# pairlab/leibnizgym

Measured on AMD Instinct MI355X. Metric: env-steps/sec (whole node), trifinger_difficulty_4 @65536 envs, 1/2/4/8 GPUs, higher is better.
Workload: dtype f32

## Files before the change

### leibnizgym_amd/csrc/tf_roles.h

```cpp
#pragma once
#include <type_traits>

#include "tf_contact.h"

#define NT 256

enum { M_ACT_IN = 1, M_RESETS = 2, M_TORQUE = 4, M_SIM = 8, M_POST = 16, M_FINISH = 32, M_ACT_RAND = 64  };
#define M_FUSED_STEP (M_ACT_IN | M_RESETS | M_TORQUE | M_SIM | M_POST | M_FINISH)
#define M_FUSED_STEP_RAND (M_FUSED_STEP | M_ACT_RAND)
#define M_FUSED_RESET (M_RESETS | M_TORQUE | M_SIM | M_POST)

#define L_REC(f) (30 * (f))
#define R_A 0
#define R_DIR 6
#define R_RXD 15
#define R_U 24
#define R_DL 27
#define P_AW 0
#define P_BW 3
#define P_MINV 6
#define P_S1 12
#define P_C1 13
#define P_P2 14
#define P_P3 17
#define P_VQ 20
#define L_POSE_A 23
#define L_POSE_B 53
#define L_WALL 90
#define L_PARK(f) L_REC(f)
#define PK_FC 0
#define PK_LINK 4
#define PK_TF 5
#define PK_TW 8
#define PK_TAU 11
#define PK_FT 14
#define L_VQFF 138
#define L_INIT 147
#define L_DR0 32
#define LDS_SLOTS 159
DEV constexpr int ffm_mbox(int fd, int k, bool boxw = false) {
    return boxw ? 180 + 6 * fd + k
         : fd == 0 ? (k == 0 ? 147 : 149 + k)
         : fd == 1 ? (k == 0 ? 148 : (k == 1 ? 59 : 153 + k))
                   : 83 + k;
}
#define NT_HELP 512
#define L_HELP_OWN 159
#define L_HELP_DR 177
#define LDS_SLOTS_HELP 180
DEV constexpr int ffm_own_mbox(int fm, int k) { return L_HELP_OWN + 6 * fm + k; }
#define L_POSE_S 150
#define LDS_SLOTS_BOX 159
#define LDS_SLOTS_BOX_WIDE 198
#define L_CONE 180
#define LDS_SLOTS_SURF 268
#define L_XCH (MAX_STATES)
#define L_NAN (MAX_STATES + 18)
#define L_VSQ (MAX_STATES + 22)
#define L_OTERM (MAX_STATES + 31)
static_assert(MAX_STATES + 37 <= LDS_SLOTS, "post-phase LDS map");
#define LD(slot) lds[(slot) * WAVE + lane]

struct Ctx {
    int tid, lane, role;
    int wave_first, i, n_valid;
    bool valid;
};

#define ST_RSRC() __builtin_amdgcn_make_buffer_rsrc((void*)P.state, 0, TF_STATE_ROWS * P.N * 4, 0x00020000)
#define LDST(row) __builtin_bit_cast(float, __builtin_amdgcn_raw_buffer_load_b32(ST_RSRC(), (unsigned)cx.i * 4u, (row) * P.N * 4, 0))
#define STST(row, val) do { if (cx.valid) __builtin_amdgcn_raw_buffer_store_b32(__builtin_bit_cast(unsigned, (float)(val)), ST_RSRC(), (unsigned)cx.i * 4u, (row) * P.N * 4, 0); } while (0)
#define BAR() __syncthreads()
#define IN_FLIGHT3(a, b, c) asm volatile("" : "+v"(a), "+v"(b), "+v"(c))
#define IN_FLIGHT4(a, b, c, d) asm volatile("" : "+v"(a), "+v"(b), "+v"(c), "+v"(d))

#ifdef TF_PHASE_TIMING
#define TF_SCR_STRIDE 256
#define NOW() ((uint32_t)__builtin_readcyclecounter())
#define STAMP(id) do { if (cx.lane == 0) ((gu32*)P.scratch)[((size_t)blockIdx.x * 4 + cx.role) * 64 + (id)] = NOW(); } while (0)
#define STAMPV(id, val) do { if (cx.lane == 0) ((gu32*)P.scratch)[((size_t)blockIdx.x * 4 + cx.role) * 64 + (id)] = (uint32_t)(val); } while (0)
#else
#define TF_SCR_STRIDE 16
#define NOW() 0u
#define STAMP(id) do { } while (0)
#define STAMPV(id, val) do { } while (0)
#endif

#define NT_F 192
template <int W, int NTH = NT>
DEV void coop_store_tile(gfloat* __restrict__ dst, const float* lds, const Ctx& cx) {
    const unsigned total = (unsigned)(cx.n_valid * W);
    gfloat* base = dst + (size_t)cx.wave_first * (size_t)W;
    const unsigned total4 = total >> 2;
    const __amdgpu_buffer_rsrc_t tile = __builtin_amdgcn_make_buffer_rsrc((void*)base, 0, (int)(total4 * 16u), 0x00020000);
    constexpr int ITER = (16 * W + NTH - 1) / NTH;
    const unsigned last4 = total4 - 1u;
#pragma unroll
    for (int k = 0; k < ITER; ++k) {
        const unsigned idx = (unsigned)cx.tid + (unsigned)(NTH * k);
        const unsigned src = (idx < last4) ? idx : last4;
        u32x4 vv = *reinterpret_cast<const u32x4*>(&lds[src * 4u]);
        __builtin_amdgcn_raw_buffer_store_b128(vv, tile, idx * 16u, 0, 0);
    }
    const unsigned tail = (total4 << 2) + (unsigned)cx.tid;
    if (tail < total) base[tail] = lds[tail];
}
template <int W, int LS, int NTH = NT>
DEV void coop_store_tile_strided(gfloat* __restrict__ dst, const float* lds, const Ctx& cx) {
    const unsigned total = (unsigned)(cx.n_valid * W);
    gfloat* base = dst + (size_t)cx.wave_first * (size_t)W;
    const unsigned total4 = total >> 2;
    const __amdgpu_buffer_rsrc_t tile = __builtin_amdgcn_make_buffer_rsrc((void*)base, 0, (int)(total4 * 16u), 0x00020000);
    constexpr int ITER = (16 * W + NTH - 1) / NTH;
    const unsigned lastf = total - 1u;
#pragma unroll
    for (int k = 0; k < ITER; ++k) {
        const unsigned idx = (unsigned)cx.tid + (unsigned)(NTH * k);
        u32x4 vv;
#pragma unroll
        for (int e = 0; e < 4; ++e) {
            unsigned g = idx * 4u + (unsigned)e;
            g = (g < lastf) ? g : lastf;
            const unsigned row = g / (unsigned)W, col = g - row * (unsigned)W;
            vv[e] = __builtin_bit_cast(unsigned, lds[row * (unsigned)LS + col]);
        }
        __builtin_amdgcn_raw_buffer_store_b128(vv, tile, idx * 16u, 0, 0);
    }
    const unsigned tail = (total4 << 2) + (unsigned)cx.tid;
    if (tail < total) { const unsigned row = tail / (unsigned)W, col = tail - row * (unsigned)W; base[tail] = lds[row * (unsigned)LS + col]; }
}
template <int A>
DEV void coop_load_tile(const float* __restrict__ src, float* lds, const Ctx& cx) {
    const float* base = src + (size_t)cx.wave_first * (size_t)A;
    const unsigned last = (unsigned)(cx.n_valid * A) - 1u;
    constexpr int ITER = (WAVE * A + NT - 1) / NT;
    float t[ITER];
#pragma unroll
    for (int k = 0; k < ITER; ++k) {
        const unsigned idx = (unsigned)cx.tid + (unsigned)(NT * k);
        t[k] = base[idx < last ? idx : last];
    }
#pragma unroll
    for (int k = 0; k < ITER; ++k) {
        const unsigned idx = (unsigned)cx.tid + (unsigned)(NT * k);
        if (idx < (unsigned)(WAVE * A)) lds[idx] = t[k];
    }
}

template <int A>
DEV void draw_action_tile(const DevParams& P, const StepArgs& sa, float* lds, const Ctx& cx) {
    constexpr int NB = (A + 3) / 4;
    for (int t = cx.tid; t < WAVE * NB; t += NT) {
        const int e = t / NB, b = t - e * NB;
        const int ge = cx.wave_first + ((e < cx.n_valid) ? e : (cx.n_valid - 1));
        float u[4];
        rng4(P, (uint32_t)(P.env_id_offset + ge), sa.frame0, RNG_ACTION + (uint32_t)b, u);
#pragma unroll
        for (int k = 0; k < 4; ++k) {
            const int c = 4 * b + k;
            if (c < A) lds[e * A + c] = 2.0f * u[k] - 1.0f;
        }
    }
}

DEV void sample_xy(float u_r, float u_t, float r_max, float& x, float& y) {
    float radius = f_sqrt(u_r) * r_max;
    float s, c;
    tf_sincos(6.2831855f * u_t, s, c);
    x = radius * c;
    y = radius * s;
}
DEV void sample_yaw_quat(float u, float q[4]) {
    float s, c;
    tf_sincos((6.2831855f * u) * 0.5f, s, c);
    q[0] = 0.0f; q[1] = 0.0f; q[2] = s; q[3] = c;
}
DEV void normalize_quat(const float n[4], float q[4]) {
    float nrm = f_sqrt(n[0] * n[0] + n[1] * n[1] + n[2] * n[2] + n[3] * n[3]);
    float inv = 1.0f / f_max(nrm, 1e-12f);
#pragma unroll
    for (int i = 0; i < 4; ++i) q[i] = n[i] * inv;
}

DEV void sample_goal_pos(const DevParams& P, uint32_t gid, uint32_t count, float xyz[3], float quat[4]) {
    const int d = P.task_difficulty;
    float u[4];
    rng4(P, gid, count, RNG_GOAL_POS, u);
    float x = 0.0f, y = 0.0f, z;
    quat[0] = 0.0f; quat[1] = 0.0f; quat[2] = 0.0f; quat[3] = 1.0f;
    if (d == -1 || d == 1 || d == 3 || d == 4 || d == 5) sample_xy(u[0], u[1], P.m.obj_max_com_dist, x, y);
    if (d == -1 || d == 1) z = P.m.obj_min_height;
    else if (d == 2 || d == 6) z = P.m.obj_min_height + 0.05f;
    else if (d == 3) z = P.m.obj_span_min_height * u[2] + P.m.obj_min_height;
    else z = P.m.obj_span_radius * u[2] + P.m.obj_radius_3d;
    if (d == -1) sample_yaw_quat(u[3], quat);
    xyz[0] = x; xyz[1] = y; xyz[2] = z;
}
DEV bool goal_has_random_quat(const DevParams& P) { const int d = P.task_difficulty; return d == 4 || d == 5 || d == 6; }
DEV void sample_goal_rot(const DevParams& P, uint32_t gid, uint32_t count, float quat[4], float gw[3]) {
    if (goal_has_random_quat(P)) {
        float v[4], n[4];
        rng4(P, gid, count, RNG_GOAL_QUAT, v);
        box_muller(v[0], v[1], n[0], n[1]);
        box_muller(v[2], v[3], n[2], n[3]);
        normalize_quat(n, quat);
    }
    if (P.goal_rotation_activate) {
        float v[4], n[4];
        rng4(P, gid, count, RNG_GOAL_ANGVEL, v);
        box_muller(v[0], v[1], n[0], n[1]);
        box_muller(v[2], v[3], n[2], n[3]);
        float nrm = f_sqrt(n[0] * n[0] + n[1] * n[1] + n[2] * n[2]);
        float mag = n[3] * P.goal_rate;
#pragma unroll
        for (int i = 0; i < 3; ++i) gw[i] = mag * (n[i] / nrm);
    } else {
        gw[0] = 0.0f; gw[1] = 0.0f; gw[2] = 0.0f;
    }
}
template <bool EXT>
DEV void goal_from_raw(const float raw[10], const float dr[TF_NUM_DR], float gp[3], float gq[4], float gw[3]) {
    gp[0] = EXT ? raw[0] + dr[TF_DR_STAGE_POS] : raw[0]; gp[1] = EXT ? raw[1] + dr[TF_DR_STAGE_POS + 1] : raw[1]; gp[2] = raw[2];
#pragma unroll
    for (int i = 0; i < 4; ++i) gq[i] = raw[3 + i];
#pragma unroll
    for (int i = 0; i < 3; ++i) gw[i] = raw[7 + i];
}
template <bool EXT>
DEV void sample_goal(const DevParams& P, uint32_t gid, uint32_t count, const float dr[TF_NUM_DR], float gp[3], float gq[4], float gw[3]) {
    float raw[10];
    sample_goal_pos(P, gid, count, &raw[0], &raw[3]);
    sample_goal_rot(P, gid, count, &raw[3], &raw[7]);
    goal_from_raw<EXT>(raw, dr, gp, gq, gw);
}

template <bool EXT>
DEV void draw_dr(const DevParams& P, uint32_t gid, uint32_t count, float dr[TF_NUM_DR]) {
    float u[4];
    rng4(P, gid, count, RNG_DR, u);
    dr[0] = FMA(P.dr_cube_mass[1] - P.dr_cube_mass[0], u[0], P.dr_cube_mass[0]);
    dr[1] = FMA(P.dr_cube_size[1] - P.dr_cube_size[0], u[1], P.dr_cube_size[0]);
    dr[2] = FMA(P.dr_friction[1] - P.dr_friction[0], u[2], P.dr_friction[0]);
    dr[3] = FMA(P.dr_motor[1] - P.dr_motor[0], u[3], P.dr_motor[0]);
    rng4(P, gid, count, RNG_DR + 1u, u);
    dr[4] = FMA(P.dr_link_mass[1] - P.dr_link_mass[0], u[0], P.dr_link_mass[0]);
    dr[5] = FMA(P.dr_restitution[1] - P.dr_restitution[0], u[1], P.dr_restitution[0]);
    if (!EXT) return;
    rng4(P, gid, count, RNG_DR + 2u, u);
#pragma unroll
    for (int k = 0; k < 3; ++k) dr[TF_DR_BASE_POS + k] = P.dr_base_pos[k] * (2.0f * u[k] - 1.0f);
    dr[TF_DR_STAGE_POS] = P.dr_stage_pos[0] * (2.0f * u[3] - 1.0f);
    rng4(P, gid, count, RNG_DR + 3u, u);
    dr[TF_DR_STAGE_POS + 1] = P.dr_stage_pos[1] * (2.0f * u[0] - 1.0f);
    dr[TF_DR_FRICTION_ROBOT] = FMA(P.dr_friction_robot[1] - P.dr_friction_robot[0], u[1], P.dr_friction_robot[0]);
    dr[TF_DR_FRICTION_OBJECT] = FMA(P.dr_friction_object[1] - P.dr_friction_object[0], u[2], P.dr_friction_object[0]);
    dr[TF_DR_FRICTION_STAGE] = FMA(P.dr_friction_stage[1] - P.dr_friction_stage[0], u[3], P.dr_friction_stage[0]);
}
DEV float pair_factor(float mu_a, float fa1, float mu_b, float fb1) {
    const float inv = 1.0f / (mu_a + mu_b);
    return FMA(mu_b * inv, fb1, FMA(mu_a * inv, fa1, 1.0f));
}

DEV float emit_scaled(float x, float lo, float hi, bool nrm, float co) {
    const float o_ = (lo + hi) * 0.5f, i_ = 1.0f / (hi - lo);
    return f_clamp(nrm ? FMA(x, 2.0f * i_, -(2.0f * o_) * i_) : x, -co, co);
}
DEV float emit_table(const DevParams& P, int col, float x, bool nrm, float co) {
    const float off = P.tables[TAB_OFF + col], inv = P.tables[TAB_INV + col];
    return f_clamp(nrm ? FMA(x, 2.0f * inv, -(2.0f * off) * inv) : x, -co, co);
}
#define QLO(j) (((j) % 3 == 0) ? -0.33f : (((j) % 3 == 1) ? 0.0f : -2.7f))
#define QHI(j) (((j) % 3 == 0) ? 1.0f : (((j) % 3 == 1) ? 1.57f : 0.0f))
#define PLO(j) (((j) == 2) ? 0.0f : -0.3f)
#define TLO(j) (((j) < 2) ? -0.4f : (((j) == 2) ? 0.0f : (((j) < 7) ? -1.0f : -0.2f)))
#define THI(j) (((j) < 2) ? 0.4f : (((j) == 2) ? 0.5f : (((j) < 7) ? 1.0f : 0.2f)))

DEV float norm3d(const float a[3], const float b[3]) {
    float dx = a[0] - b[0], dy = a[1] - b[1], dz = a[2] - b[2];
    return f_sqrt(dx * dx + dy * dy + dz * dz);
}
DEV float ipow(float x, int n) {
    float t = x;
    for (int k = 1; k < n; ++k) t = t * x;
    return t;
}
DEV float norm_p3(const float a[3], const float b[3], int p) {
    if (__builtin_expect(p == 2, 1)) return norm3d(a, b);
    const float ax = f_abs(a[0] - b[0]), ay = f_abs(a[1] - b[1]), az = f_abs(a[2] - b[2]);
    if (p == 1) return (ax + ay) + az;
    if (p == TF_NORM_INF) return f_max(f_max(ax, ay), az);
    const float mx = f_max(f_max(ax, ay), az);
    if (!(mx > 0.0f)) return 0.0f;
    const float s = (ipow(ax / mx, p) + ipow(ay / mx, p)) + ipow(az / mx, p);
    float y = tf_exp(tf_log(s) / (float)p);
    const float yp1 = ipow(y, p - 1);
    y = y - (yp1 * y - s) / ((float)p * yp1);
    return mx * y;
}

DEV void tip_state(const DevModel& m, const Yaw& y, const FK& k, const float q[3], const float qd[3], float out[13]) {
    float To[3];
    link_point<3>(k, m.tip_origin, To);
    base_to_world(y, To, &out[0]);
    float sy, cy, sx, cxx;
    tf_sincos(0.5f * q[0], sy, cy);
    tf_sincos(0.5f * (q[1] + q[2]), sx, cxx);
    float qyx[4] = {cy * sx, sy * cxx, -(sy * sx), cy * cxx};
    float qz[4] = {0.0f, 0.0f, y.hs, y.hc};
    quat_mul(qz, qyx, &out[3]);
    float L1[3], L2[3], L3[3], vb[3], wb[3];
    levers(k, To, L1, L2, L3);
#pragma unroll
    for (int i = 0; i < 3; ++i) vb[i] = L1[i] * qd[0] + L2[i] * qd[1] + L3[i] * qd[2];
    wb[0] = k.ax[0] * qd[1] + k.ax[0] * qd[2];
    wb[1] = qd[0];
    wb[2] = k.ax[2] * qd[1] + k.ax[2] * qd[2];
    dir_base_to_world(y, vb, &out[7]);
    dir_base_to_world(y, wb, &out[10]);
}

struct FingerPubRegs { FK k; };
DEV void read_pub(const float* lds, int lane, int f, FingerPubRegs& p) {
    const int pb = L_REC(f);
#pragma unroll
    for (int j = 0; j < 3; ++j) { p.k.p2[j] = LD(pb + P_P2 + j); p.k.p3[j] = LD(pb + P_P3 + j); }
#pragma unroll
    for (int j = 0; j < 6; ++j) p.k.Minv[j] = LD(pb + P_MINV + j);
    p.k.s1 = LD(pb + P_S1); p.k.c1 = LD(pb + P_C1);
    p.k.ax[0] = p.k.c1; p.k.ax[1] = 0.0f; p.k.ax[2] = -p.k.s1;
}

struct TipContact {
    bool active;
    float J[9], Dinv[3], bias, lam[3], mu;
    float arm[3];
};

template <int A, bool IS_RESET, bool ASYM, int MODE, int X, bool WIDE, bool HELP = false, bool DR = true>
DEV void finger_role(const DevParams& P, const StepArgs& sa, const float* __restrict__ action, float* lds, const Ctx& cx) {
    static_assert(!HELP || WIDE, "helper wavefronts: 256-register kernels only");
    constexpr bool EXT = X != 0;
    constexpr bool BOXK = X == 2;
    const DevModel& m = P.m;
    const int f = cx.role, lane = cx.lane;
    constexpr int OD = TF_OBS_DIM_BASE + A, SD = OD + TF_STATES_EXTRA;
    constexpr int TW = ASYM ? SD : OD;
    constexpr int NDR = EXT ? TF_NUM_DR : TF_DR_BASE_POS;
    constexpr int AJ = A / 3;
    const Yaw yw = {m.base_yaw_cos[f], m.base_yaw_sin[f], m.base_half_yaw_cos[f], m.base_half_yaw_sin[f], m.base_height};
    const uint32_t gid = (uint32_t)(P.env_id_offset + cx.i);
    float q[3], qd[3], tau[3], dr[TF_NUM_DR];
    uint8_t fl_reset = 0;
    uint32_t fl_count = 0;
// ... 1109 lines not shown
struct StatsTicket { unsigned long long mine, old; };
DEV void stats_begin(const DevParams& P, const LaneStats& st, int lane, StatsTicket& tk) {
    float vals[11];
#pragma unroll
    for (int t = 0; t < 6; ++t) vals[t] = st.rew[t];
    vals[6] = st.pos_cnt; vals[7] = st.ori_cnt; vals[8] = st.succ; vals[9] = st.resets; vals[10] = st.nonfinite;
    float sum = 0.0f;
#pragma unroll
    for (int k = 0; k < 11; ++k) {
        const float s = wave_sum_lane63(vals[k]);
        const float b = __builtin_bit_cast(float, __builtin_amdgcn_readlane(__builtin_bit_cast(int, s), WAVE - 1));
        sum = (lane == k) ? b : sum;
    }
    const long long fx = (long long)((double)sum * STAT_FIX);
    tk.mine = ((unsigned long long)fx << STAT_COUNT_BITS) + 1ull;
    tk.old = 0ull;
    const int shard = (int)blockIdx.x & (STAT_SHARDS - 1);
    gu64* acc = (gu64*)P.tickets;
    if (lane < 11)
        tk.old = __hip_atomic_fetch_add(&acc[(shard * 11 + lane) * STAT_STRIDE], tk.mine, __ATOMIC_RELAXED, __HIP_MEMORY_SCOPE_AGENT);
}
DEV void stats_end(const DevParams& P, int lane, const StatsTicket& tk) {
    const unsigned long long cmask = (1ull << STAT_COUNT_BITS) - 1ull;
    const int nw = (int)gridDim.x;
    const int shard = (int)blockIdx.x & (STAT_SHARDS - 1);
    const unsigned long long members = (unsigned long long)((nw - shard + STAT_SHARDS - 1) / STAT_SHARDS);
    const unsigned long long nshards = (unsigned long long)(nw < STAT_SHARDS ? nw : STAT_SHARDS);
    gu64* acc = (gu64*)P.tickets;
    if (lane < 11 && (tk.old & cmask) == members - 1ull) {
        const unsigned long long total1 = tk.old + tk.mine;
        __hip_atomic_store(&acc[(shard * 11 + lane) * STAT_STRIDE], 0ull, __ATOMIC_RELAXED, __HIP_MEMORY_SCOPE_AGENT);
        const unsigned long long v2 = (total1 & ~cmask) + 1ull;
        gu64* top = &acc[(STAT_SHARDS * 11 + lane) * STAT_STRIDE];
        const unsigned long long old2 = __hip_atomic_fetch_add(top, v2, __ATOMIC_RELAXED, __HIP_MEMORY_SCOPE_AGENT);
        if ((old2 & cmask) == nshards - 1ull) {
            __hip_atomic_store(top, 0ull, __ATOMIC_RELAXED, __HIP_MEMORY_SCOPE_AGENT);
            const long long fxs = (long long)(old2 + v2) >> STAT_COUNT_BITS;
            const float total = (float)((double)fxs / STAT_FIX);
            const int k = lane;
            const float o = (k < 6 || k == 8) ? total / (float)P.N : total;
            const int slot = (k < 6) ? k : ((k == 6) ? TF_INFO_POS_COUNT : ((k == 7) ? TF_INFO_ORI_COUNT :
                             ((k == 8) ? TF_INFO_SUCCESS_MEAN : ((k == 9) ? TF_INFO_NUM_RESETS : TF_INFO_NUM_NONFINITE))));
            P.info[slot] = o;
        }
    }
}

DEV void stats_zero(LaneStats& st) {
#pragma unroll
    for (int t = 0; t < 6; ++t) st.rew[t] = 0.0f;
    st.pos_cnt = 0.0f; st.ori_cnt = 0.0f; st.succ = 0.0f; st.resets = 0.0f; st.nonfinite = 0.0f;
}


DEV void ld_row(const float* lds, int lane, int rb, float2v rec[3]) {
#pragma unroll
    for (int j = 0; j < 3; ++j) { rec[j].x = LD(rb + j); rec[j].y = LD(rb + 3 + j); }
}
DEV float pk_row_vel_lds(const float* lds, int lane, int rb, const Twist& t) { float2v rec[3]; ld_row(lds, lane, rb, rec); return pk_row_vel(rec, t); }
DEV void pk_row_apply_lds(const float* lds, int lane, int rb, float dl, float2v mI, Twist& t) { float2v rec[3]; ld_row(lds, lane, rb, rec); pk_row_apply(rec, dl, mI, t); }

DEV void wall_arms(bool box, const float* lds, int lane, const float r[3], const float n[2], float a[3], float b[3], float c3[3]) {
    wall_arm_n(r, n, a);
    wall_arm_t(r, n, b);
    c3[0] = 0.0f; c3[1] = 0.0f; c3[2] = 0.0f;
    if (__builtin_expect(box, 0)) {
        float S[6], t[3], ez[3];
#pragma unroll
        for (int e = 0; e < 6; ++e) S[e] = LD(L_POSE_S + e);
        sym3_mul(S, a, t); a[0] = t[0]; a[1] = t[1]; a[2] = t[2];
        sym3_mul(S, b, t); b[0] = t[0]; b[1] = t[1]; b[2] = t[2];
        box_axis(0, ez);
        box_arm(S, r, ez, c3);
    }
}

template <int A, bool IS_RESET, bool ASYM, int MODE, int X, bool WIDE, bool HELP = false, bool SURF = false, bool DR = true>
DEV void cube_role(const DevParams& P, const StepArgs& sa, const float* __restrict__ action, float* lds, const Ctx& cx) {
    constexpr bool EXT = X != 0;
    constexpr bool BOXK = X == 2;
    static_assert(!SURF || (WIDE && !BOXK), "the surface normal of the cube corners is built into the 256-register cube kernels only");
    const DevModel& m = P.m;
    const int lane = cx.lane;
    constexpr int OD = TF_OBS_DIM_BASE + A, SD = OD + TF_STATES_EXTRA;
    constexpr int TW = ASYM ? SD : OD;
    constexpr int NDR = EXT ? TF_NUM_DR : TF_DR_BASE_POS;
    const uint32_t gid = (uint32_t)(P.env_id_offset + cx.i);
    float cp[3], cq[4], cv[3], cw[3], dr[TF_NUM_DR];
    float lam_cf[12], lam_cw[12], cf_face = 0.0f, cw_face = 0.0f;
    uint8_t fl_reset = 0, fl_goal_reset = 0, fl_successes = 0;
    int fl_steps = 0;
    uint32_t fl_count = 0;
    STAMP(0);
#pragma unroll
    for (int j = 0; j < 3; ++j) { cp[j] = LDST(TF_S_CUBE_P + j); cv[j] = LDST(TF_S_CUBE_V + j); cw[j] = LDST(TF_S_CUBE_W + j); }
#pragma unroll
    for (int j = 0; j < 4; ++j) cq[j] = LDST(TF_S_CUBE_Q + j);
#pragma unroll
    for (int j = 0; j < TF_NUM_DR; ++j) dr[j] = (DR && j < NDR && P.dr_enable) ? LDST(TF_S_DR + j) : TF_DR_NEUTRAL(j);
    if (MODE & (M_RESETS | M_POST | M_FINISH)) {
        fl_reset = P.reset_buf[(unsigned)cx.i];
        fl_goal_reset = P.goal_reset_buf[(unsigned)cx.i];
        fl_successes = P.successes[(unsigned)cx.i];
        fl_steps = (int)P.steps[(unsigned)cx.i];
        fl_count = P.reset_count[(unsigned)cx.i];
    }
    if (MODE & M_ACT_RAND) draw_action_tile<A>(P, sa, lds, cx);
    else if (MODE & M_ACT_IN) coop_load_tile<A>(action, lds, cx);
    else if (MODE & (M_RESETS | M_TORQUE | M_POST)) coop_load_tile<A>((const float*)P.action_buf, lds, cx);
    if (DR && P.dr_enable) {
#pragma unroll
        for (int j = 0; j < NDR; ++j) LD(L_DR0 + j) = dr[j];
    }
    BAR();
    if (!(MODE & (M_ACT_IN | M_RESETS))) BAR();
    STAMP(1);
    if (MODE & (M_SIM | M_RESETS)) {
        cf_face = LDST(TF_S_CF_FACE); cw_face = LDST(TF_S_CW_FACE);
#pragma unroll
        for (int j = 0; j < 12; ++j) { lam_cf[j] = LDST(TF_S_LAM_CF + j); lam_cw[j] = 0.0f; }
        const bool cw_was = cw_face != 0.0f;
        if (__builtin_amdgcn_ballot_w64(cw_was) != 0ull) {
#pragma unroll
            for (int j = 0; j < 12; ++j) { const float t = LDST(TF_S_LAM_CW + j); lam_cw[j] = cw_was ? t : 0.0f; }
        }
    }
    bool c_reset = fl_reset != 0, c_goal_reset = fl_goal_reset != 0, c_successes = fl_successes != 0;
    int c_steps = fl_steps;
    float n_resets = 0.0f;
    if (MODE & M_RESETS) {
        const bool rflag = IS_RESET || (fl_reset != 0);
        const bool gflag = !IS_RESET && (fl_goal_reset != 0);
        uint32_t count = fl_count;
        float gp[3] = {0.0f, 0.0f, 0.0f}, gq[4] = {0.0f, 0.0f, 0.0f, 0.0f}, gw[3] = {0.0f, 0.0f, 0.0f};
        float nx_obj[4] = {0.0f, 0.0f, 0.0f, 0.0f}, nx_goal[10] = {0.0f, 0.0f, 0.0f, 0.0f, 0.0f, 0.0f, 0.0f, 0.0f, 0.0f, 0.0f};
        bool have = false;
        if (!IS_RESET && __builtin_amdgcn_ballot_w64(rflag) != 0ull) {
            const uint32_t tag = __builtin_bit_cast(uint32_t, LDST(TF_S_NEXT_TAG));
            have = rflag && (tag == count + 1u);
#pragma unroll
            for (int j = 0; j < 4; ++j) nx_obj[j] = LDST(TF_S_NEXT_OBJ + j);
#pragma unroll
            for (int j = 0; j < 10; ++j) nx_goal[j] = LDST(TF_S_NEXT_GOAL + j);
        }
        const bool draw_now = __builtin_amdgcn_ballot_w64(rflag && !have) != 0ull;
        if (rflag) {
            if (DR && P.dr_enable) draw_dr<EXT>(P, gid, count, dr);
            if (P.object_reset_type == TF_RESET_DEFAULT) {
                cp[0] = EXT ? 0.0f + dr[TF_DR_STAGE_POS] : 0.0f; cp[1] = EXT ? 0.0f + dr[TF_DR_STAGE_POS + 1] : 0.0f; cp[2] = m.obj_min_height * dr[1];
                cq[0] = 0.0f; cq[1] = 0.0f; cq[2] = 0.0f; cq[3] = 1.0f;
#pragma unroll
                for (int k = 0; k < 3; ++k) { cv[k] = 0.0f; cw[k] = 0.0f; }
            } else if (P.object_reset_type == TF_RESET_RANDOM) {
                float ox = nx_obj[0], oy = nx_obj[1], oq[4] = {0.0f, 0.0f, nx_obj[2], nx_obj[3]};
                if (draw_now) {
                    float u[4], tx, ty, tq[4];
                    rng4(P, gid, count, RNG_OBJECT, u);
                    sample_xy(u[0], u[1], m.obj_max_com_dist, tx, ty);
                    sample_yaw_quat(u[2], tq);
                    ox = have ? ox : tx; oy = have ? oy : ty; oq[2] = have ? oq[2] : tq[2]; oq[3] = have ? oq[3] : tq[3];
                }
                cp[0] = EXT ? ox + dr[TF_DR_STAGE_POS] : ox; cp[1] = EXT ? oy + dr[TF_DR_STAGE_POS + 1] : oy;
                cp[2] = m.obj_min_height * dr[1];
#pragma unroll
                for (int k = 0; k < 4; ++k) cq[k] = oq[k];
#pragma unroll
                for (int k = 0; k < 3; ++k) { cv[k] = 0.0f; cw[k] = 0.0f; }
            }
            if (draw_now) {
                float raw[10];
                sample_goal_pos(P, gid, count, &raw[0], &raw[3]);
                sample_goal_rot(P, gid, count, &raw[3], &raw[7]);
#pragma unroll
                for (int j = 0; j < 10; ++j) nx_goal[j] = have ? nx_goal[j] : raw[j];
            }
            goal_from_raw<EXT>(nx_goal, dr, gp, gq, gw);
            count = count + 1u;
#pragma unroll
            for (int j = 0; j < 12; ++j) { lam_cf[j] = 0.0f; lam_cw[j] = 0.0f; }
            cf_face = 0.0f; cw_face = 0.0f;
            n_resets = cx.valid ? 1.0f : 0.0f;
        }
        if (gflag) {
            sample_goal<EXT>(P, gid, count, dr, gp, gq, gw);
            count = count + 1u;
        }
        if (cx.valid) {
            if (rflag) { P.reset_buf[(unsigned)cx.i] = 0; P.steps[(unsigned)cx.i] = 0; P.successes[(unsigned)cx.i] = 0; }
            if (gflag) P.goal_reset_buf[(unsigned)cx.i] = 0;
            if (rflag || gflag) P.reset_count[(unsigned)cx.i] = count;
        }
        if (DR && rflag && P.dr_enable) {
#pragma unroll
            for (int j = 0; j < NDR; ++j) STST(TF_S_DR + j, dr[j]);
        }
        if (rflag || gflag) {
#pragma unroll
            for (int j = 0; j < 3; ++j) { STST(TF_S_GOAL_P + j, gp[j]); STST(TF_S_GOAL_W + j, gw[j]); }
#pragma unroll
            for (int j = 0; j < 4; ++j) STST(TF_S_GOAL_Q + j, gq[j]);
        }
        c_reset = false;
        c_goal_reset = IS_RESET ? (fl_goal_reset != 0) : false;
        c_successes = rflag ? false : (fl_successes != 0);
        c_steps = rflag ? 0 : fl_steps;
    }
    if (MODE & (M_ACT_IN | M_RESETS)) {
        BAR();
        BAR();
        coop_store_tile<A>(P.action_buf, lds, cx);
    }
    if (MODE & M_TORQUE) {
#pragma unroll
        for (int j = 0; j < 3; ++j) STST(TF_S_PREV_OBJ_P + j, cp[j]);
#pragma unroll
        for (int j = 0; j < 4; ++j) STST(TF_S_PREV_OBJ_Q + j, cq[j]);
    }
    STAMP(2);
    if (MODE & M_SIM) {
        const float h = P.hsub, inv_h = 1.0f / h;
        const int nsub = sa.nsim * P.substeps;
        __builtin_amdgcn_s_setprio(3);
#pragma unroll
        for (int c = 0; c < 4; ++c) {
#pragma unroll
            for (int d = 0; d < 3; ++d) LD(L_WALL + 12 * c + 9 + d) = lam_cw[3 * c + d];
        }
        for (int s = 0; s < nsub; ++s) {
            const int sb_ = 4 + 12 * (s & 1);
            (void)sb_;
            float drs[TF_NUM_DR];
#pragma unroll
            for (int j = 0; j < TF_NUM_DR; ++j) drs[j] = (!DR || WIDE || j >= NDR || s == 0 || !P.dr_enable) ? dr[j] : LDST(TF_S_DR + j);
            const float* dr = drs;
            const float cube_mass = m.cube_mass * dr[0];
            const float cube_inertia = m.cube_inertia * dr[0] * dr[1] * dr[1];
            const float inv_m = 1.0f / cube_mass, inv_I = 1.0f / cube_inertia;
            const float fr1 = dr[TF_DR_FRICTION_ROBOT] - 1.0f, fo1 = dr[TF_DR_FRICTION_OBJECT] - 1.0f, fs1 = dr[TF_DR_FRICTION_STAGE] - 1.0f;
            const float mu_fc = (m.mu_finger_cube * dr[2]) * (EXT ? pair_factor(m.mu_robot, fr1, m.mu_object, fo1) : 1.0f);
            const float mu_cf = (m.mu_cube_floor * dr[2]) * (EXT ? pair_factor(m.mu_object, fo1, m.mu_floor, fs1) : 1.0f);
            const float mu_cw = (m.mu_cube_wall * dr[2]) * (EXT ? pair_factor(m.mu_object, fo1, m.mu_stage, fs1) : 1.0f);
            const float soff[2] = {dr[TF_DR_STAGE_POS], dr[TF_DR_STAGE_POS + 1]};
            const float rest_ff = m.restitution_ff * dr[5];
            const float ws = m.warm_start;
            constexpr bool box = BOXK;
            float hc[3];
#pragma unroll
            for (int j = 0; j < 3; ++j) hc[j] = (box ? m.box_half[j] : m.cube_half) * dr[1];
            float v[3], w[3];
            float R[9];
            quat_to_rot(cq, R);
            {
                float wf[3] = {cw[0], cw[1], cw[2]};
                if (__builtin_expect(box && m.box_gyroscopic, 0)) {
                    float wb[3], Iw[3], tq[3];
                    mat3T_mul(R, wf, wb);
#pragma unroll
                    for (int k = 0; k < 3; ++k) Iw[k] = m.box_inertia[k] * wb[k];
                    cross3(Iw, wb, tq);
#pragma unroll
                    for (int k = 0; k < 3; ++k) wb[k] = FMA(h, tq[k] / m.box_inertia[k], wb[k]);
                    mat3_mul(R, wb, wf);
                }
                float dl = 1.0f - h * m.cube_linear_damping, da = 1.0f - h * m.cube_angular_damping;
#pragma unroll
                for (int j = 0; j < 3; ++j) {
                    v[j] = FMA(h, P.grav[j], cv[j]) * dl;
                    w[j] = wf[j] * da;
                }
                if (__builtin_expect(box, 0)) {
                    float sc[3], si[3], S[6], Sinv[6], wh[3];
#pragma unroll
                    for (int k = 0; k < 3; ++k) { sc[k] = f_sqrt(m.cube_inertia / m.box_inertia[k]); si[k] = 1.0f / sc[k]; }
                    rot_diag_rot(R, sc, S);
                    rot_diag_rot(R, si, Sinv);
                    sym3_mul(Sinv, w, wh);
#pragma unroll
                    for (int j = 0; j < 3; ++j) w[j] = wh[j];
#pragma unroll
                    for (int e = 0; e < 6; ++e) LD(L_POSE_S + e) = S[e];
                }
            }
#pragma unroll
            for (int j = 0; j < 3; ++j) { LD(L_POSE_A + j) = cp[j]; LD(L_POSE_B + j) = v[j]; LD(L_POSE_B + 3 + j) = w[j]; }
#pragma unroll
            for (int j = 0; j < 4; ++j) LD(L_POSE_A + 3 + j) = cq[j];
            float fr_[12], fDinv[12], fbias[4], flam[12];
            if constexpr (!WIDE) {
#include "tf_floor_corners.inc"
            }
            bool wall_lane = false;
            bool slot_any[4] = {false, false, false, false};
            unsigned cone_any = 0u;
            constexpr bool WREG = WIDE && !BOXK;
            float w_r[6], w_n[4], w_D[6], w_bias[2], w_lam[6], w_a[6], w_b[6];
            if constexpr (!HELP) {
#include "tf_wall_corners.inc"
            }
            STAMP(sb_ + 0);
            BAR();
            STAMP(sb_ + 1);
            if constexpr (HELP) {
#include "tf_wall_corners.inc"
            } else {
#include "tf_ff_distal.inc"
            }
            if (!WIDE && m.ff_middle_pairs != 0) {
                const TfLinkShape& sh = m.shape2;
                const float jx = m.j3_origin[0], jy = m.j3_origin[1], jz = m.j3_origin[2];
                const float inv_j = f_rcp(FMA(jy, jy, jz * jz));
#pragma unroll 1
                for (int o_ = 2; o_ >= (BOXK ? 1 : 2); --o_)
#pragma unroll 1
                for (int fm = 0; fm < 3; ++fm) {
                    FingerPubRegs pm;
                    read_pub(lds, lane, fm, pm);
                    const Yaw ym = {m.base_yaw_cos[fm], m.base_yaw_sin[fm], 0.0f, 0.0f, m.base_height};
                    const float ex[3] = {pm.k.c1, 0.0f, -pm.k.s1};
                    float ey[3], aw[3], bw[3];
                    {
                        float g[3], xg[3], ez[3], ab[3], bb[3];
#pragma unroll
                        for (int i = 0; i < 3; ++i) g[i] = FMA(-jx, ex[i], pm.k.p3[i] - pm.k.p2[i]);
                        cross3(ex, g, xg);
#pragma unroll
                        for (int i = 0; i < 3; ++i) { ey[i] = FMA(jy, g[i], -(jz * xg[i])) * inv_j; ez[i] = FMA(jz, g[i], jy * xg[i]) * inv_j; }
#pragma unroll
                        for (int i = 0; i < 3; ++i) {
                            ab[i] = FMA(sh.a[2], ez[i], FMA(sh.a[1], ey[i], FMA(sh.a[0], ex[i], pm.k.p2[i])));
                            bb[i] = FMA(sh.b[2], ez[i], FMA(sh.b[1], ey[i], FMA(sh.b[0], ex[i], pm.k.p2[i])));
                        }
                        base_to_world(ym, ab, aw);
                        base_to_world(ym, bb, bw);
                    }
                    {
                        const int o = o_;
                        const int fd = (fm + o >= 3) ? fm + o - 3 : fm + o;
                        float Pm[3], Pd[3], sp;
                        {
                            float Ad[3], Bd[3];
#pragma unroll
                            for (int j = 0; j < 3; ++j) { Ad[j] = LD(L_REC(fd) + P_AW + j); Bd[j] = LD(L_REC(fd) + P_BW + j); }
                            seg_seg_s(aw, bw, Ad, Bd, Pm, Pd, sp);
                        }
                        const float dv[3] = {Pd[0] - Pm[0], Pd[1] - Pm[1], Pd[2] - Pm[2]};
                        const float dist2 = dot3(dv, dv);
                        const float inv = f_rsqrt(f_max(dist2, 1e-12f));
                        const float dist = dist2 * inv;
                        const float n[3] = {dv[0] * inv, dv[1] * inv, dv[2] * inv};
                        float nm[3];
                        dir_world_to_base(ym, n, nm);
                        const float u1 = dot3(nm, ex), u2 = dot3(nm, ey);
                        const float rho = FMA(sp, sh.rho[1] - sh.rho[0], sh.rho[0]);
                        const float h1 = FMA(sp, sh.w1[1] - sh.w1[0], sh.w1[0]) - rho, h2 = FMA(sp, sh.w2[1] - sh.w2[0], sh.w2[0]) - rho;
                        const float o1 = FMA(sp, sh.o1[1] - sh.o1[0], sh.o1[0]), o2 = FMA(sp, sh.o2[1] - sh.o2[0], sh.o2[0]);
                        const float ext = FMA(o2, u2, FMA(o1, u1, FMA(h2, f_abs(u2), FMA(h1, f_abs(u1), rho))));
                        const float gap = dist - ext - m.cap_radius;
                        if ((dist2 > 1e-12f) && (gap < m.contact_margin)) {
                            float Jd[3], Wd[3], Jm[3], Wm[3], vd[3], vm[3];
                            {
                                const Yaw yd = {m.base_yaw_cos[fd], m.base_yaw_sin[fd], 0.0f, 0.0f, m.base_height};
                                FingerPubRegs pd;
                                read_pub(lds, lane, fd, pd);
                                float C[3], Cb_[3], L1[3], L2[3], L3[3], nb[3];
#pragma unroll
                                for (int j = 0; j < 3; ++j) C[j] = FMA(-m.cap_radius, n[j], Pd[j]);
                                world_to_base(yd, C, Cb_);
                                levers(pd.k, Cb_, L1, L2, L3);
                                dir_world_to_base(yd, n, nb);
                                Jd[0] = dot3(L1, nb); Jd[1] = dot3(L2, nb); Jd[2] = dot3(L3, nb);
                                sym3_mul(pd.k.Minv, Jd, Wd);
                            }
                            {
                                float C[3], Cb_[3], L1[3], L2[3], L3[3];
#pragma unroll
                                for (int j = 0; j < 3; ++j) C[j] = FMA(ext, n[j], Pm[j]);
                                world_to_base(ym, C, Cb_);
                                levers(pm.k, Cb_, L1, L2, L3);
                                Jm[0] = dot3(L1, nm); Jm[1] = dot3(L2, nm); Jm[2] = 0.0f;
                                sym3_mul(pm.k.Minv, Jm, Wm);
                            }
#pragma unroll
                            for (int j = 0; j < 3; ++j) { vd[j] = LD(L_REC(fd) + P_VQ + j); vm[j] = LD(L_REC(fm) + P_VQ + j); }
                            const float vn0 = dot3(Jd, vd) - dot3(Jm, vm);
                            if (contact_live(m, gap, vn0, h)) {
                                const float bias = contact_bias(m, gap, vn0, inv_h, rest_ff);
                                const float lam = f_max(-(vn0 + bias) * f_rcp2(dot3(Jd, Wd) + dot3(Jm, Wm)), 0.0f);
#pragma unroll
                                for (int j = 0; j < 3; ++j) {
                                    const float dd = Wd[j] * lam, dm = Wm[j] * lam;
                                    if (dd != 0.0f) LD(L_VQFF + 3 * fd + j) = LD(L_VQFF + 3 * fd + j) + dd;
                                    if (dm != 0.0f) LD(L_VQFF + 3 * fm + j) = LD(L_VQFF + 3 * fm + j) - dm;
                                }
                            }
                        }
                    }
                }
            }
            STAMP(sb_ + 2);
            BAR();
            STAMP(sb_ + 3);
            if constexpr (WIDE) {
#include "tf_floor_corners.inc"
            }
            STAMP(sb_ + 4);
            BAR();
            STAMP(sb_ + 5);
            if constexpr (WIDE && !BOXK) {
            Twist tw;
#pragma unroll
            for (int j = 0; j < 3; ++j) { tw.p[j].x = v[j]; tw.p[j].y = w[j]; }
            float2v mI; mI.x = inv_m; mI.y = inv_I;
            float cDinv[9], cbias[3], clam[9], Km[9];
            float2v rec[27];
#pragma unroll
            for (int f = 0; f < 3; ++f) {
                const int rb = L_REC(f);
                cbias[f] = LD(L_INIT + f);
#pragma unroll
                for (int d = 0; d < 3; ++d) { cDinv[3 * f + d] = LD(L_VQFF + 3 * f + d); clam[3 * f + d] = LD(rb + R_DL + d); Km[3 * f + d] = LD(rb + R_A + d); }
#pragma unroll
                for (int j = 0; j < 9; ++j) { rec[9 * f + j].x = LD(rb + R_DIR + j); rec[9 * f + j].y = LD(rb + R_RXD + j); }
                if (cDinv[3 * f] > 0.0f) {
#pragma unroll
                    for (int d = 0; d < 3; ++d) pk_row_apply_neg(&rec[9 * f + 3 * d], clam[3 * f + d], mI, tw);
                }
            }
#pragma unroll
            for (int c = 0; c < 4; ++c) {
                if (fDinv[3 * c] > 0.0f) {
                    cz_apply(&fr_[3 * c], flam[3 * c], mI, tw);
                    cx_apply(&fr_[3 * c], flam[3 * c + 1], mI, tw);
                    cy_apply(&fr_[3 * c], flam[3 * c + 2], mI, tw);
                }
            }
#pragma unroll
            for (int c = 0; c < 4; ++c) {
                const int wb = L_WALL + 12 * c;
                if (c < 2) {
                    if (slot_any[c] && w_D[3 * c] > 0.0f) {
                        wn_apply(&w_n[2 * c], &w_a[3 * c], w_lam[3 * c], mI, tw);
                        wt_apply(&w_n[2 * c], &w_b[3 * c], w_lam[3 * c + 1], mI, tw);
                        cz_apply(&w_r[3 * c], w_lam[3 * c + 2], mI, tw);
                    }
                } else if (slot_any[c] && LD(wb + 5) > 0.0f) {
                    float r[3] = {LD(wb), LD(wb + 1), LD(wb + 2)}, n[2] = {LD(wb + 3), LD(wb + 4)};
                    float a[3], b[3];
                    wall_arm_n(r, n, a);
                    wall_arm_t(r, n, b);
                    wn_apply(n, a, LD(wb + 9), mI, tw);
                    wt_apply(n, b, LD(wb + 10), mI, tw);
                    cz_apply(r, LD(wb + 11), mI, tw);
                }
            }
            if constexpr (SURF) {
                if (__builtin_expect(cone_any != 0u, 0)) {
#pragma unroll 1
                    for (int c = 0; c < 4; ++c) {
                        const int cb = L_CONE + 22 * c, wb = L_WALL + 12 * c;
                        if (((cone_any >> c) & 1u) && LD(cb + 18) > 0.0f) {
#pragma unroll 1
                            for (int d = 0; d < 3; ++d) pk_row_apply_lds(lds, lane, cb + 6 * d, LD(wb + 9 + d), mI, tw);
                        }
                    }
                }
            }
            uint32_t t_wait = 0u, t_fc = 0u, t_floor = 0u;
            STAMP(sb_ + 9);
            for (int it = 0; it < P.iters; ++it) {
                const uint32_t tf0_ = NOW();
                const bool last = it == P.iters - 1;
                float uu[9];
#pragma unroll
                for (int f = 0; f < 3; ++f) {
#pragma unroll
                    for (int j = 0; j < 3; ++j) uu[3 * f + j] = LD(L_REC(f) + R_U + j);
                }
#pragma unroll
                for (int f = 0; f < 3; ++f) {
#ifdef TF_DIAG_NO_FC
                    if (false) {
#else
                    if (cDinv[3 * f] > 0.0f) {
#endif
                        const int rb = L_REC(f);
                        const float2v* R = &rec[9 * f];
                        float vr[3], dl[3];
                        {
                            float2v p0 = R[0] * tw.p[0], p1 = R[3] * tw.p[0], p2 = R[6] * tw.p[0];
                            p0 = pk_fma(R[1], tw.p[1], p0); p1 = pk_fma(R[4], tw.p[1], p1); p2 = pk_fma(R[7], tw.p[1], p2);
                            p0 = pk_fma(R[2], tw.p[2], p0); p1 = pk_fma(R[5], tw.p[2], p1); p2 = pk_fma(R[8], tw.p[2], p2);
                            vr[0] = uu[3 * f] - (p0.x + p0.y); vr[1] = uu[3 * f + 1] - (p1.x + p1.y); vr[2] = uu[3 * f + 2] - (p2.x + p2.y);
                        }
                        dl[0] = solve_normal(clam[3 * f], cDinv[3 * f], vr[0], cbias[f]);
                        vr[1] = FMA(Km[3 * f], dl[0], vr[1]);
                        dl[1] = solve_tangent(clam[3 * f + 1], cDinv[3 * f + 1], vr[1], mu_fc * clam[3 * f]);
                        vr[2] = FMA(Km[3 * f + 2], dl[1], FMA(Km[3 * f + 1], dl[0], vr[2]));
                        dl[2] = solve_tangent(clam[3 * f + 2], cDinv[3 * f + 2], vr[2], mu_fc * clam[3 * f]);
#pragma unroll
                        for (int d = 0; d < 3; ++d) {
                            LD(rb + R_DL + d) = dl[d];
                            pk_row_apply_neg(&R[3 * d], dl[d], mI, tw);
                        }
                    }
                }
                t_fc += NOW() - tf0_;
                { const uint32_t t0_ = NOW(); BAR(); t_wait += NOW() - t0_; }
#pragma unroll
                for (int c = 0; c < 4; ++c) {
                    const float* r = &fr_[3 * c];
#ifdef TF_DIAG_NO_FLOOR
                    if (false) {
#else
                    if (fDinv[3 * c] > 0.0f) {
#endif
                        float dl = solve_normal(flam[3 * c], fDinv[3 * c], cz_vrel(r, tw), fbias[c]);
                        cz_apply(r, dl, mI, tw);
                        dl = solve_tangent(flam[3 * c + 1], fDinv[3 * c + 1], cx_vrel(r, tw), mu_cf * flam[3 * c]);
                        cx_apply(r, dl, mI, tw);
                        dl = solve_tangent(flam[3 * c + 2], fDinv[3 * c + 2], cy_vrel(r, tw), mu_cf * flam[3 * c]);
                        cy_apply(r, dl, mI, tw);
                    }
                }
                t_floor += NOW() - tf0_;
#pragma unroll
                for (int c = 0; c < 4; ++c) {
#ifdef TF_DIAG_NO_WALL
                    continue;
#endif
                    if (!slot_any[c]) continue;
                    const int wb = L_WALL + 12 * c;
                    if (c < 2) {
                        float dl = solve_normal(w_lam[3 * c], w_D[3 * c], wn_vrel(&w_n[2 * c], &w_a[3 * c], tw), w_bias[c]);
                        wn_apply(&w_n[2 * c], &w_a[3 * c], dl, mI, tw);
                        dl = solve_tangent(w_lam[3 * c + 1], w_D[3 * c + 1], wt_vrel(&w_n[2 * c], &w_b[3 * c], tw), mu_cw * w_lam[3 * c]);
                        wt_apply(&w_n[2 * c], &w_b[3 * c], dl, mI, tw);
                        dl = solve_tangent(w_lam[3 * c + 2], w_D[3 * c + 2], cz_vrel(&w_r[3 * c], tw), mu_cw * w_lam[3 * c]);
                        cz_apply(&w_r[3 * c], dl, mI, tw);
                        if (last && w_D[3 * c] > 0.0f) {
#pragma unroll
                            for (int d = 0; d < 3; ++d) LD(wb + 9 + d) = w_lam[3 * c + d];
                        }
                    } else {
                        float r[3] = {LD(wb), LD(wb + 1), LD(wb + 2)}, n[2] = {LD(wb + 3), LD(wb + 4)};
                        float Dinv[3] = {LD(wb + 5), LD(wb + 6), LD(wb + 7)}, bias = LD(wb + 8);
                        float lam[3] = {LD(wb + 9), LD(wb + 10), LD(wb + 11)};
                        float a[3], b[3];
                        wall_arm_n(r, n, a);
                        wall_arm_t(r, n, b);
                        float dl = solve_normal(lam[0], Dinv[0], wn_vrel(n, a, tw), bias);
                        wn_apply(n, a, dl, mI, tw);
                        dl = solve_tangent(lam[1], Dinv[1], wt_vrel(n, b, tw), mu_cw * lam[0]);
                        wt_apply(n, b, dl, mI, tw);
                        dl = solve_tangent(lam[2], Dinv[2], cz_vrel(r, tw), mu_cw * lam[0]);
                        cz_apply(r, dl, mI, tw);
                        if (Dinv[0] > 0.0f) {
#pragma unroll
                            for (int d = 0; d < 3; ++d) LD(wb + 9 + d) = lam[d];
                        }
                    }
                }
                if constexpr (SURF) {
                    if (__builtin_expect(cone_any != 0u, 0)) {
#pragma unroll
                    for (int c = 0; c < 4; ++c) {
                        const int cb = L_CONE + 22 * c, wb = L_WALL + 12 * c;
                        if (((cone_any >> c) & 1u) && LD(cb + 18) > 0.0f) {
                            float lim = 0.0f;
#pragma unroll
                            for (int d = 0; d < 3; ++d) {
                                const float vr = pk_row_vel_lds(lds, lane, cb + 6 * d, tw);
                                float lam = LD(wb + 9 + d);
                                const float dl = (d == 0) ? solve_normal(lam, LD(cb + 18), vr, LD(cb + 21)) : solve_tangent(lam, LD(cb + 18 + d), vr, lim);
                                lim = (d == 0) ? mu_cw * lam : lim;
                                LD(wb + 9 + d) = lam;
                                pk_row_apply_lds(lds, lane, cb + 6 * d, dl, mI, tw);
                            }
                        }
                    }
                    }
                }
                if (last) {
#pragma unroll
                    for (int f = 0; f < 3; ++f) {
                        const int rb = L_REC(f);
                        float ftv[3] = {0.0f, 0.0f, 0.0f}, Fc[3] = {0.0f, 0.0f, 0.0f};
                        if (cDinv[3 * f] > 0.0f) {
#pragma unroll
                            for (int j = 0; j < 3; ++j) {
                                ftv[j] = FMA(rec[9 * f + 6 + j].x, clam[3 * f + 2], rec[9 * f + 3 + j].x * clam[3 * f + 1]);
                                Fc[j] = FMA(rec[9 * f + j].x, clam[3 * f], ftv[j]) * inv_h;
                            }
                        }
                        LD(L_INIT + f) = clam[3 * f];
#pragma unroll
                        for (int j = 0; j < 3; ++j) { LD(rb + R_A + j) = ftv[j]; LD(rb + R_A + 3 + j) = Fc[j]; }
                    }
                }
                { const uint32_t t0_ = NOW(); BAR(); t_wait += NOW() - t0_; }
            }
            STAMP(sb_ + 6);
            STAMPV(sb_ + 8, t_wait);
            STAMPV(sb_ + 10, t_fc);
            STAMPV(sb_ + 11, t_floor);
#pragma unroll
            for (int j = 0; j < 3; ++j) { v[j] = tw.p[j].x; w[j] = tw.p[j].y; }
            } else {
            float cDinv[9], cbias[3], clam[9];
            constexpr int NRR = WIDE ? 27 : 1, NRA = WIDE ? 9 : 1;
            float rA[NRA], rDir[NRR], rRxd[NRR];
// ... 503 lines not shown
```

Baseline: 1.010 billion.

## Fuse finger-finger distal and middle contact passes into one loop for non-box path

For the non-wide, non-box-kernel variant, replaces the separate distal finger-finger pass and the middle-link pass with a single per-pair loop that computes both contacts together, reusing loaded segment endpoints and kinematics. Middle-link impulses are held back in spare LDS slots and applied at the end so the update order stays consistent. A compile-time check guards against collisions with those slots, and two live registers are spilled to LDS around the pass. The aim is fewer LDS reloads and loop iterations, at the cost of more code and register pressure in one fused body.

```diff
diff --git a/leibnizgym_amd/csrc/tf_ff_pass.inc b/leibnizgym_amd/csrc/tf_ff_pass.inc
--- /dev/null
+++ b/leibnizgym_amd/csrc/tf_ff_pass.inc
@@ -0,0 +1,175 @@
+#pragma unroll
+            for (int f = 0; f < 3; ++f) {
+#pragma unroll
+                for (int j = 0; j < 3; ++j) LD(L_VQFF + 3 * f + j) = LD(L_REC(f) + P_VQ + j);
+            }
+            {
+                const bool ffm_on = m.ff_middle_pairs != 0;
+                TfLinkShape sh = {};
+                float jx = 0.0f, jy = 0.0f, jz = 0.0f, inv_j = 0.0f;
+                if (ffm_on) {
+                    sh = m.shape2;
+                    jx = m.j3_origin[0]; jy = m.j3_origin[1]; jz = m.j3_origin[2];
+                    inv_j = f_rcp(FMA(jy, jy, jz * jz));
+                }
+                auto side_row = [&](const FK& k, const Yaw& yy, const float C[3], const float nb[3], bool joint3, float J[3], float W[3]) __attribute__((always_inline)) {
+                    float Cb_[3], L1[3], L2[3], L3[3];
+                    world_to_base(yy, C, Cb_);
+                    levers(k, Cb_, L1, L2, L3);
+                    J[0] = dot3(L1, nb); J[1] = dot3(L2, nb); J[2] = joint3 ? dot3(L3, nb) : 0.0f;
+                    sym3_mul(k.Minv, J, W);
+                };
+                auto seg_seg_sel = [&](const float p1[3], const float q1[3], const float p2[3], const float q2[3], float c1[3], float c2[3], float& s_out) __attribute__((always_inline)) {
+                    const float d1[3] = {q1[0] - p1[0], q1[1] - p1[1], q1[2] - p1[2]};
+                    const float d2[3] = {q2[0] - p2[0], q2[1] - p2[1], q2[2] - p2[2]};
+                    const float r[3] = {p1[0] - p2[0], p1[1] - p2[1], p1[2] - p2[2]};
+                    const float a = dot3(d1, d1), e = dot3(d2, d2), f = dot3(d2, r), c = dot3(d1, r), b = dot3(d1, d2);
+                    const float denom = FMA(a, e, -(b * b));
+                    const float ia = f_rcp(a), ie = f_rcp(e);
+                    const float s_in = f_clamp(FMA(b, f, -(c * e)) * f_rcp(denom), 0.0f, 1.0f);
+                    const float s_lo = f_clamp(-c * ia, 0.0f, 1.0f), s_hi = f_clamp((b - c) * ia, 0.0f, 1.0f);
+                    float s = (denom > 1e-12f) ? s_in : 0.0f;
+                    float t = FMA(b, s, f) * ie;
+                    const bool lo = t < 0.0f, hi = t > 1.0f;
+                    s = lo ? s_lo : (hi ? s_hi : s);
+                    t = lo ? 0.0f : (hi ? 1.0f : t);
+#pragma unroll
+                    for (int i = 0; i < 3; ++i) { c1[i] = FMA(s, d1[i], p1[i]); c2[i] = FMA(t, d2[i], p2[i]); }
+                    s_out = s;
+                };
+#pragma unroll 1
+                for (int p = 0; p < 3; ++p) {
+                    const int fa = p, fb = (p == 2) ? 0 : p + 1, fd = (p == 0) ? 2 : p - 1;
+                    const Yaw ya = {m.base_yaw_cos[fa], m.base_yaw_sin[fa], 0.0f, 0.0f, m.base_height};
+                    float Aa[3], Ba[3], Ab[3], Bb[3], Ad[3], Bd[3];
+                    FK ka;
+#pragma unroll
+                    for (int j = 0; j < 3; ++j) { Aa[j] = LD(L_REC(fa) + P_AW + j); Ba[j] = LD(L_REC(fa) + P_BW + j); Ab[j] = LD(L_REC(fb) + P_AW + j); Bb[j] = LD(L_REC(fb) + P_BW + j); }
+#pragma unroll
+                    for (int j = 0; j < 3; ++j) { ka.p2[j] = LD(L_REC(fa) + P_P2 + j); ka.p3[j] = LD(L_REC(fa) + P_P3 + j); }
+                    ka.s1 = LD(L_REC(fa) + P_S1); ka.c1 = LD(L_REC(fa) + P_C1);
+#pragma unroll
+                    for (int j = 0; j < 3; ++j) { Ad[j] = LD(L_REC(fd) + P_AW + j); Bd[j] = LD(L_REC(fd) + P_BW + j); }
+                    __builtin_amdgcn_sched_barrier(0);
+                    float Pa[3], Pb[3], sa_;
+                    seg_seg_sel(Aa, Ba, Ab, Bb, Pa, Pb, sa_);
+                    const float dv[3] = {Pa[0] - Pb[0], Pa[1] - Pb[1], Pa[2] - Pb[2]};
+                    const float dist2 = dot3(dv, dv);
+                    const float inv = f_rsqrt(f_max(dist2, 1e-12f));
+                    const float dist = dist2 * inv;
+                    const float gap = dist - 2.0f * m.cap_radius;
+                    const float ex[3] = {ka.c1, 0.0f, -ka.s1};
+                    float ey[3], aw[3], bw[3];
+                    {
+                        float g[3], xg[3], ez[3], ab[3], bb[3];
+#pragma unroll
+                        for (int i = 0; i < 3; ++i) g[i] = FMA(-jx, ex[i], ka.p3[i] - ka.p2[i]);
+                        cross3(ex, g, xg);
+#pragma unroll
+                        for (int i = 0; i < 3; ++i) { ey[i] = FMA(jy, g[i], -(jz * xg[i])) * inv_j; ez[i] = FMA(jz, g[i], jy * xg[i]) * inv_j; }
+#pragma unroll
+                        for (int i = 0; i < 3; ++i) {
+                            ab[i] = FMA(sh.a[2], ez[i], FMA(sh.a[1], ey[i], FMA(sh.a[0], ex[i], ka.p2[i])));
+                            bb[i] = FMA(sh.b[2], ez[i], FMA(sh.b[1], ey[i], FMA(sh.b[0], ex[i], ka.p2[i])));
+                        }
+                        base_to_world(ya, ab, aw);
+                        base_to_world(ya, bb, bw);
+                    }
+                    float Pm[3], Pd[3], sp;
+                    seg_seg_sel(aw, bw, Ad, Bd, Pm, Pd, sp);
+                    const float dvm[3] = {Pd[0] - Pm[0], Pd[1] - Pm[1], Pd[2] - Pm[2]};
+                    const float dist2m = dot3(dvm, dvm);
+                    const float invm = f_rsqrt(f_max(dist2m, 1e-12f));
+                    const float distm = dist2m * invm;
+                    const float nw[3] = {dvm[0] * invm, dvm[1] * invm, dvm[2] * invm};
+                    float nm[3];
+                    dir_world_to_base(ya, nw, nm);
+                    const float u1 = dot3(nm, ex), u2 = dot3(nm, ey);
+                    const float rho = FMA(sp, sh.rho[1] - sh.rho[0], sh.rho[0]);
+                    const float h1 = FMA(sp, sh.w1[1] - sh.w1[0], sh.w1[0]) - rho, h2 = FMA(sp, sh.w2[1] - sh.w2[0], sh.w2[0]) - rho;
+                    const float o1 = FMA(sp, sh.o1[1] - sh.o1[0], sh.o1[0]), o2 = FMA(sp, sh.o2[1] - sh.o2[0], sh.o2[0]);
+                    const float ext = FMA(o2, u2, FMA(o1, u1, FMA(h2, f_abs(u2), FMA(h1, f_abs(u1), rho))));
+                    const float gapm = distm - ext - m.cap_radius;
+                    float dd[3] = {-0.0f, -0.0f, -0.0f}, dm[3] = {0.0f, 0.0f, 0.0f};
+                    if (ffm_on && (dist2m > 1e-12f) && (gapm < m.contact_margin)) {
+                        float Jd[3], Wd[3], Jm[3], Wm[3], vd[3], vm[3], C[3];
+                        {
+                            const Yaw yd = {m.base_yaw_cos[fd], m.base_yaw_sin[fd], 0.0f, 0.0f, m.base_height};
+                            FingerPubRegs pd;
+                            read_pub(lds, lane, fd, pd);
+                            float nb[3];
+#pragma unroll
+                            for (int j = 0; j < 3; ++j) C[j] = FMA(-m.cap_radius, nw[j], Pd[j]);
+                            dir_world_to_base(yd, nw, nb);
+                            side_row(pd.k, yd, C, nb, true, Jd, Wd);
+                        }
+#pragma unroll
+                        for (int j = 0; j < 3; ++j) C[j] = FMA(ext, nw[j], Pm[j]);
+                        {
+                            FingerPubRegs pm;
+                            read_pub(lds, lane, fa, pm);
+                            side_row(pm.k, ya, C, nm, false, Jm, Wm);
+                        }
+#pragma unroll
+                        for (int j = 0; j < 3; ++j) { vd[j] = LD(L_REC(fd) + P_VQ + j); vm[j] = LD(L_REC(fa) + P_VQ + j); }
+                        const float vn0 = dot3(Jd, vd) - dot3(Jm, vm);
+                        if (contact_live(m, gapm, vn0, h)) {
+                            const float bias = contact_bias(m, gapm, vn0, inv_h, rest_ff);
+                            const float lam = f_max(-(vn0 + bias) * f_rcp2(dot3(Jd, Wd) + dot3(Jm, Wm)), 0.0f);
+#pragma unroll
+                            for (int j = 0; j < 3; ++j) {
+                                const float d = Wd[j] * lam;
+                                dd[j] = (d != 0.0f) ? d : -0.0f;
+                                dm[j] = Wm[j] * lam + 0.0f;
+                            }
+                        }
+                    }
+                    if ((dist2 > 1e-12f) && (gap < m.contact_margin)) {
+                        const float n[3] = {dv[0] * inv, dv[1] * inv, dv[2] * inv};
+                        float Ja[3], Wa[3], Jb[3], Wb[3], va[3], vb[3], C[3], nb[3];
+#pragma unroll
+                        for (int j = 0; j < 3; ++j) C[j] = FMA(-m.cap_radius, n[j], Pa[j]);
+                        dir_world_to_base(ya, n, nb);
+                        {
+                            FingerPubRegs pa;
+                            read_pub(lds, lane, fa, pa);
+                            side_row(pa.k, ya, C, nb, true, Ja, Wa);
+                        }
+                        {
+                            const Yaw yb = {m.base_yaw_cos[fb], m.base_yaw_sin[fb], 0.0f, 0.0f, m.base_height};
+                            FingerPubRegs pb;
+                            read_pub(lds, lane, fb, pb);
+#pragma unroll
+                            for (int j = 0; j < 3; ++j) C[j] = FMA(m.cap_radius, n[j], Pb[j]);
+                            dir_world_to_base(yb, n, nb);
+                            side_row(pb.k, yb, C, nb, true, Jb, Wb);
+                        }
+#pragma unroll
+                        for (int j = 0; j < 3; ++j) { va[j] = LD(L_VQFF + 3 * fa + j); vb[j] = LD(L_VQFF + 3 * fb + j); }
+                        const float vn0 = dot3(Ja, va) - dot3(Jb, vb);
+                        if (contact_live(m, gap, vn0, h)) {
+                            const float bias = contact_bias(m, gap, vn0, inv_h, rest_ff);
+                            const float lam = f_max(-(vn0 + bias) * f_rcp2(dot3(Ja, Wa) + dot3(Jb, Wb)), 0.0f);
+#pragma unroll
+                            for (int j = 0; j < 3; ++j) {
+                                LD(L_VQFF + 3 * fa + j) = FMA(Wa[j], lam, va[j]);
+                                LD(L_VQFF + 3 * fb + j) = FMA(-Wb[j], lam, vb[j]);
+                            }
+                        }
+                    }
+                    if (p == 0) {
+#pragma unroll
+                        for (int j = 0; j < 3; ++j) { LD(ffh_slot(0, j)) = dd[j]; LD(ffh_slot(0, 3 + j)) = dm[j]; }
+                    } else if (p == 1) {
+#pragma unroll
+                        for (int j = 0; j < 3; ++j) { LD(ffh_slot(1, j)) = dd[j]; LD(L_VQFF + 3 + j) = LD(L_VQFF + 3 + j) - dm[j]; }
+                    } else {
+#pragma unroll
+                        for (int j = 0; j < 3; ++j) {
+                            LD(L_VQFF + 3 + j) = LD(L_VQFF + 3 + j) + dd[j];
+                            LD(L_VQFF + 6 + j) = (LD(L_VQFF + 6 + j) + LD(ffh_slot(0, j))) - dm[j];
+                            LD(L_VQFF + j) = (LD(L_VQFF + j) - LD(ffh_slot(0, 3 + j))) + LD(ffh_slot(1, j));
+                        }
+                    }
+                }
+            }
diff --git a/leibnizgym_amd/csrc/tf_roles.h b/leibnizgym_amd/csrc/tf_roles.h
--- a/leibnizgym_amd/csrc/tf_roles.h
+++ b/leibnizgym_amd/csrc/tf_roles.h
@@ -49,6 +49,25 @@
 #define L_HELP_DR 177
 #define LDS_SLOTS_HELP 180
 DEV constexpr int ffm_own_mbox(int fm, int k) { return L_HELP_OWN + 6 * fm + k; }
+DEV constexpr int ffh_slot(int row, int k) {
+    return row == 0 ? (k < 5 ? 147 + k : 155)
+                    : 83 + k;
+}
+DEV constexpr bool ffh_slots_clear() {
+    for (int row = 0; row < 2; ++row)
+        for (int k = 0; k < (row == 0 ? 6 : 3); ++k) {
+            const int s = ffh_slot(row, k);
+            for (int fd = 0; fd < 3; ++fd) {
+                for (int c = 3; c < 6; ++c) if (s == ffm_mbox(fd, c)) return false;
+                if (s >= L_REC(fd) && s < L_REC(fd) + 23) return false;
+            }
+            if ((s >= L_POSE_A && s < L_POSE_A + 7) || (s >= L_POSE_B && s < L_POSE_B + 6) || (s >= L_WALL && s < L_VQFF + 9) || s >= LDS_SLOTS) return false;
+            for (int row2 = 0; row2 < 2; ++row2)
+                for (int k2 = 0; k2 < (row2 == 0 ? 6 : 3); ++k2) if ((row2 != row || k2 != k) && s == ffh_slot(row2, k2)) return false;
+        }
+    return true;
+}
+static_assert(ffh_slots_clear(), "hold-back slots of the finger-finger pass");
 #define L_POSE_S 150
 #define LDS_SLOTS_BOX 159
 #define LDS_SLOTS_BOX_WIDE 198
@@ -1764,10 +1783,14 @@
             STAMP(sb_ + 1);
             if constexpr (HELP) {
 #include "tf_wall_corners.inc"
+            } else if constexpr (!WIDE && !BOXK) {
+                LD(89) = flam[11]; LD(59) = flam[10];
+#include "tf_ff_pass.inc"
+                flam[11] = LD(89); flam[10] = LD(59);
             } else {
 #include "tf_ff_distal.inc"
             }
-            if (!WIDE && m.ff_middle_pairs != 0) {
+            if (!WIDE && BOXK && m.ff_middle_pairs != 0) {
                 const TfLinkShape& sh = m.shape2;
                 const float jx = m.j3_origin[0], jy = m.j3_origin[1], jz = m.j3_origin[2];
                 const float inv_j = f_rcp(FMA(jy, jy, jz * jz));
```

New measurement: 1.009 billion, median of 2. No clear change (-0.2%).
